# jbrea/BayesianOptimization.jl

Hardware: AMD Instinct MI355X
Metric: acquisition-candidates/sec (N=3000,d=8) (higher is better)
Workload: dtype f64

## Files before the change

### bayesianoptimization.jl_amd/csrc/bohip.hip

```cpp
#include "../../include/bohip.h"
#include "../../include/bohip_paths.h"
#include "../../include/bohip_fit.h"
#include "../../include/bohip_qei.h"
#include "../../include/bohip_acq.h"
#include "../../include/bohip_kg.h"
#include "../../include/bohip_ens.h"
#include "kernels_linalg.hip"
#include "kernels_chol.hip"
#include "kernels_exec.hip"
#include "kernels_score.hip"
#include "kernels_batch.hip"
#include "kernels_sample.hip"
#include "kernels_qei.hip"
#include "kernels_kg.hip"
#include "kernels_path.hip"
#include "kernels_ascent.hip"
#include "kernels_fit.hip"
#include "kernels_ens.hip"
#include "kernels_small.hip"
#include "direct_l.h"

#include <algorithm>
#include <atomic>
#include <chrono>
// ... 292 lines not shown
    HIPCHK(hipMalloc(&g->dr, (g->ld + 256) * 8));
    HIPCHK(hipMalloc(&g->dt, (g->ld + 256) * 8));
    HIPCHK(hipMalloc(&g->dApp, (size_t)APP_ROWS * g->ld * 8));
    {
        const size_t Tm = (size_t)(g->ld / TILE) + 1;
        HIPCHK(hipMalloc(&g->dchol_flags, chol_flag_words((int)std::min<size_t>(Tm, CHOL_DF_TCAP)) * sizeof(unsigned)));
        HIPCHK(hipMalloc(&g->dchol_idl, Tm * CH_PANELS * 256 * 8));
    }
    HIPCHK(hipMemsetAsync(g->dL, 0, mat, g->stream));
    HIPCHK(hipMemsetAsync(g->dW, 0, mat, g->stream));
    HIPCHK(hipMemsetAsync(g->dWT, 0, mat, g->stream));
    HIPCHK(hipMemsetAsync(g->dS, 0, mat, g->stream));
    if (g->n > 0) {
        HIPCHK(hipMemcpyAsync(g->dX, g->hX.data(), (size_t)g->n * g->d * 8, hipMemcpyHostToDevice, g->stream));
        HIPCHK(hipMemcpyAsync(g->dy, g->hy.data(), (size_t)g->n * 8, hipMemcpyHostToDevice, g->stream));
    }
    g->stale = true;
    return 0;
}

static int g_bulk_pieces = 4;
static int g_sample_mfma_min = 200;
static int g_path_mfma_min = 24;
static int g_split = 1;
static int g_asc_wg_nmax = 256;
static const double g_asc_first_step = 0.1;
static int g_asc_fold = 1;
static int g_asc_lockstep = 0;
static int g_small_m = 0;
static int g_small_r = -1;
static int g_inv_hi_h = 16;
static int g_chol_df = 1;
static bool g_chol_df_strict = false;
static bool g_chol_df_dump = false;
static int g_chol_df_tmax = 96;
static std::atomic<int> g_chol_df_skip{0}, g_chol_df_backoff{0};
static unsigned long long g_chol_spin_ticks = CH_SPIN_TICKS_DEFAULT;
static int g_chol_exec_patience_us = 1000;
static int g_chol_exec_fill_inv = 1;
static int g_chol_exec_inv_pairs = 0;
static std::atomic<int> g_chol_inv_grp_min{28};
static std::atomic<int> g_chol_inv_g{8};
static int g_chol_nsf = 3;
static int g_chol_exec_urgent = -1;
static int g_chol_exec_second = 1;
static int g_small_zero_copy = 1;
static int g_chol_exec_nbu = 2;
static int g_chol_exec_fast = -1;
static int g_chol_exec_pairs = -1;
static int g_chol_exec_wgs = -1;
static int g_append_alpha_inc = 1;
static int64_t g_chunk_rows_forced = 0;
static int g_prune_m = -1;
static int launch_gemm_nt(bohip_gp* g, const GemmNTParams& p, int batch = 1, hipStream_t st = nullptr, bool hi = false) {
    if (p.mt <= 0 || p.nt64 <= 0 || p.kc <= 0 || batch <= 0) return 0;
    if (hi) hipLaunchKernelGGL(k_gemm_nt_hi, dim3(p.mt * p.nt64, batch), dim3(GEMM_THREADS_8), glds3_lds_bytes<4>(), st ? st : g->stream, p);
    else hipLaunchKernelGGL(k_gemm_nt, dim3(p.mt * p.nt64, batch), dim3(GEMM_THREADS_8), glds3_lds_bytes<4>(), st ? st : g->stream, p);
    HIPCHK(hipGetLastError());
    return 0;
}

static int device_cus();
static void read_dev_knobs() {
#if BOHIP_DEV_KNOBS
    struct Knob { const char* name; int* v; int lo, hi; };
    static int chunk_rows = 0, dump = 0;
    const Knob knobs[] = {
        {"BOHIP_CHOL_DF_TMAX", &g_chol_df_tmax, 0, CHOL_DF_TCAP}, {"BOHIP_INV_HI_H", &g_inv_hi_h, 0, 1 << 20},
        {"BOHIP_CHOL_EXEC_PAIRS", &g_chol_exec_pairs, -1, 64},
        {"BOHIP_CHOL_EXEC_URGENT", &g_chol_exec_urgent, 1, 1 << 20}, {"BOHIP_CHOL_NSF", &g_chol_nsf, 1, CH_NSF_MAX},
        {"BOHIP_CHOL_EXEC_PATIENCE_US", &g_chol_exec_patience_us, 0, 1 << 30}, {"BOHIP_CHOL_EXEC_FILL_INV", &g_chol_exec_fill_inv, 0, 1},
        {"BOHIP_CHOL_EXEC_INV_PAIRS", &g_chol_exec_inv_pairs, 0, 1}, {"BOHIP_CHOL_EXEC_WGS", &g_chol_exec_wgs, 1, 1 << 20},
        {"BOHIP_CHOL_EXEC_FAST", &g_chol_exec_fast, -1, 1 << 20},
        {"BOHIP_CHOL_EXEC_SECOND", &g_chol_exec_second, 0, 1}, {"BOHIP_SMALL_ZERO_COPY", &g_small_zero_copy, 0, 1}, {"BOHIP_CHOL_EXEC_NBU", &g_chol_exec_nbu, 0, 16}, {"BOHIP_CHUNK_ROWS", &chunk_rows, 0, 1 << 30},
        {"BOHIP_PRUNE_M", &g_prune_m, -1, 1 << 16},
        {"BOHIP_APPEND_ALPHA_INC", &g_append_alpha_inc, 0, 1}, {"BOHIP_BULK_PIECES", &g_bulk_pieces, 0, 8}, {"BOHIP_SPLIT", &g_split, 0, 1},
        {"BOHIP_SMALL_R", &g_small_r, 0, SMALL_MAX}, {"BOHIP_SMALL_M", &g_small_m, 0, 1 << 20}, {"BOHIP_CHOL_DF_DUMP", &dump, 0, 1},
    };
    for (const Knob& k : knobs)
        if (const char* e = getenv(k.name)) *k.v = std::min(k.hi, std::max(k.lo, atoi(e)));
    g_chunk_rows_forced = chunk_rows;
    g_chol_df_dump = dump != 0;
#endif
}

static int one_time_kernel_setup() {
    static bool done_dev[64] = {false};
    int dev = 0;
    HIPCHK(hipGetDevice(&dev));
    bool& done = done_dev[dev & 63];
    if (done) return 0;
    HIPCHK(hipFuncSetAttribute((const void*)k_potf2_inv, hipFuncAttributeMaxDynamicSharedMemorySize, POTF2_LDS_BYTES));
    HIPCHK(hipFuncSetAttribute((const void*)k_gemm_nt, hipFuncAttributeMaxDynamicSharedMemorySize, glds3_lds_bytes<4>()));
    HIPCHK(hipFuncSetAttribute((const void*)k_trigemm_sq, hipFuncAttributeMaxDynamicSharedMemorySize, glds3_lds_bytes<4>()));
    HIPCHK(hipFuncSetAttribute((const void*)k_trigemm_rows, hipFuncAttributeMaxDynamicSharedMemorySize, RS_LDS_BYTES));
    HIPCHK(hipFuncSetAttribute((const void*)k_batch_cond<true>, hipFuncAttributeMaxDynamicSharedMemorySize, BATCH_LDS_MAX));
    HIPCHK(hipFuncSetAttribute((const void*)k_batch_cond<false>, hipFuncAttributeMaxDynamicSharedMemorySize, BATCH_LDS_MAX));
    HIPCHK(hipFuncSetAttribute((const void*)k_chol_chain, hipFuncAttributeMaxDynamicSharedMemorySize, CH_LDS_BYTES));
    HIPCHK(hipFuncSetAttribute((const void*)k_gemm_nt_hi, hipFuncAttributeMaxDynamicSharedMemorySize, glds3_lds_bytes<4>()));
    HIPCHK(hipFuncSetAttribute((const void*)k_chol_exec, hipFuncAttributeMaxDynamicSharedMemorySize, glds3_lds_bytes<4>()));
    HIPCHK(hipFuncSetAttribute((const void*)k_trimv_stream<TRIMV_D>, hipFuncAttributeMaxDynamicSharedMemorySize, trimv_lds_bytes(TRIMV_D)));
    HIPCHK(hipFuncSetAttribute((const void*)k_path_mfma<true>, hipFuncAttributeMaxDynamicSharedMemorySize, (int)path_mfma_lds_bytes(DMAX)));
    HIPCHK(hipFuncSetAttribute((const void*)k_path_mfma<false>, hipFuncAttributeMaxDynamicSharedMemorySize, (int)path_mfma_lds_bytes(DMAX)));
    HIPCHK(hipFuncSetAttribute((const void*)k_kg<true>, hipFuncAttributeMaxDynamicSharedMemorySize, (int)kg_lds_bytes(KG_RMAX)));
    HIPCHK(hipFuncSetAttribute((const void*)k_kg<false>, hipFuncAttributeMaxDynamicSharedMemorySize, (int)kg_lds_bytes(KG_RMAX)));
    if (const char* e = getenv("BOHIP_CHOL_DATAFLOW")) g_chol_df = atoi(e);
    if (const char* e = getenv("BOHIP_CHOL_SPIN_US")) g_chol_spin_ticks = 100ull * (unsigned long long)std::max(1, atoi(e));
    if (const char* e = getenv("BOHIP_CHOL_INV_G")) g_chol_inv_g = std::min(64, std::max(0, atoi(e)));
    if (const char* e = getenv("BOHIP_CHOL_INV_GRP_MIN")) g_chol_inv_grp_min = std::max(0, atoi(e));
    if (const char* e = getenv("BOHIP_ASC_WG_NMAX")) g_asc_wg_nmax = std::max(0, atoi(e));
    if (const char* e = getenv("BOHIP_ASC_LOCKSTEP")) { g_asc_lockstep = atoi(e) == 1; g_asc_fold = atoi(e) != 2; }
    if (const char* e = getenv("BOHIP_SAMPLE_MFMA_MIN")) g_sample_mfma_min = std::max(1, atoi(e));
    g_chol_df_strict = getenv("BOHIP_CHOL_DF_STRICT") != nullptr;
    read_dev_knobs();
    done = true;
    return 0;
}

static int launch_rows_trimv(bohip_gp* g, const double* W, int64_t N0, const double* rows, int P, double* out, int upper);
static int compute_alpha(bohip_gp* g) {
    const int64_t N = g->n;
    g->alpha_inc_run = 0;
    hipLaunchKernelGGL(k_sub_mean, dim3((N + 255) / 256), dim3(256), 0, g->stream, g->dy, g->beta, N, g->dr);
    HIPCHK(hipGetLastError());
    CHK(launch_rows_trimv(g, g->dW, N, g->dr, 1, g->dt, 0));
    CHK(launch_rows_trimv(g, g->dWT, N, g->dt, 1, g->dalpha, 1));
    HIPCHK(hipMemcpyAsync(g->dW + N * g->ld, g->dalpha, (size_t)N * 8, hipMemcpyDeviceToDevice, g->stream));
    return 0;
}

static int check_info(bohip_gp* g) {
    int info = 0;
    if (g->hpin) {
        int* pw = reinterpret_cast<int*>(g->hpin + 3 * SMALL_R) + 1;
        HIPCHK(hipMemcpyAsync(pw, g->dinfo, sizeof(int), hipMemcpyDeviceToHost, g->stream));
        HIPCHK(hipStreamSynchronize(g->stream));
        info = *pw;
    } else {
        HIPCHK(hipMemcpyAsync(&info, g->dinfo, sizeof(int), hipMemcpyDeviceToHost, g->stream));
        HIPCHK(hipStreamSynchronize(g->stream));
    }
    if (info != 0) {
        g->pivot = info;
        g->stale = true;
        return fail(BOHIP_E_NOTPD, "kernel matrix not positive definite at pivot " + std::to_string(info));
    }
    g->pivot = 0;
// ... 1135 lines not shown
    return 0;
}

constexpr int PRUNE_K1 = 64;
constexpr int PRUNE_ROWS_CAP = 256;
constexpr int PRUNE_R2_GROUPS = 8;
constexpr int64_t PRUNE_R_MAX = 8192;
static int prune_tiles(int T) {
    if (g_prune_m >= 0) return g_prune_m < T ? g_prune_m : 0;
    int m = 2;
    while ((double)m * (m + 1) < 0.02 * T * (T + 1)) ++m;
    return m < T ? m : 0;
}
static std::vector<int> rows_halves(const std::vector<int>& pieces) {
    std::vector<int> out;
    for (int c : pieces) {
        const int rt = c & 0xffff, mode = c >> 16;
        if (mode == PIECE_UPPER_SOLO) out.push_back(rt | 1 << 17);
        else { out.push_back(rt | 1 << 16); out.push_back(rt); }
    }
    std::stable_sort(out.begin(), out.end(), [](int a, int b) {
        return 8 * (a & 0xffff) + ((a >> 16) & 1) * 4 > 8 * (b & 0xffff) + ((b >> 16) & 1) * 4;
    });
    return out;
}
static int rows_halves_from(const std::vector<int>& hv, int t0) {
    int n = 0;
    while (n < (int)hv.size() && (hv[n] & 0xffff) >= t0) ++n;
    return n;
}
static int launch_trigemm_rows(bohip_gp* g, const double* KsT, const int* halves, int NH, const int* list, const unsigned* cnt,
                               int cnt_max, double* q, int64_t ldq, double* mu, int groups = 0, const PruneFinish* pf = nullptr,
                               unsigned* arrive = nullptr) {
    if (NH <= 0 || cnt_max <= 0) return 0;
    RowsParams rp{};
    rp.W = g->dW; rp.ldw = g->ld; rp.KsT = KsT; rp.ldk = g->ld; rp.list = list; rp.cnt = cnt; rp.cnt_max = cnt_max;
    rp.halves = halves; rp.NH = NH; rp.G = groups > 0 ? groups : (cnt_max + RS_COLS - 1) / RS_COLS;
    rp.alpha_row = g->n; rp.q = q; rp.ldq = ldq; rp.mu = mu;
    if (pf) { rp.finish = 1; rp.arrive = arrive; rp.pf = *pf; }
    hipLaunchKernelGGL(k_trigemm_rows, dim3((unsigned)(8 * ((NH + 7) / 8) * rp.G)), dim3(RS_THREADS), RS_LDS_BYTES, g->stream, rp);
    HIPCHK(hipGetLastError());
    return 0;
}
static int launch_trigemm_on(bohip_gp* g, const double* KsT, const int* pieces, int NP, int CT, double* q, int64_t ldq, double* mu_raw,
                             FuseParams fz) {
    const int n_local = (CT + 7) / 8;
    if (NP <= 0 || CT <= 0) return 0;
    if (g->timing && g->dclk) fz.clk = g->dclk;
    hipLaunchKernelGGL(k_trigemm_sq, dim3(8 * n_local * NP), dim3(GEMM_THREADS_8), glds3_lds_bytes<4>(), g->stream, g->dW, g->ld, KsT,
                       g->ld, pieces, NP, CT, g->n, q, ldq, mu_raw, (int64_t)0, nullptr, g->ld, fz);
    HIPCHK(hipGetLastError());
    return 0;
}
static int pruned_pass(bohip_gp* g, const double* dXs, int64_t R, int m, const AcqParams& ap, Best* d_best, int64_t best_off,
                       double* ub_host = nullptr, bool long_form = false) {
    CHK(one_time_kernel_setup());
    if (!g->hprune_stat) {
        HIPCHK(hipHostMalloc((void**)&g->hprune_stat, 64, hipHostMallocDefault));
        g->hprune_stat[0] = 0u;
    }
    const int64_t N = g->n, Npad = round_up(N + 1, TILE), Rpad = round_up(R, TILE) + TILE, ld = g->ld;
    const int T = (int)(Npad / TILE);
    const int64_t P = Npad / 64;
    CHK(ensure_pieces(g, T, N));
    std::vector<int> pa, pb;
    for (int c : g->hpieces) ((c & 0xffff) < m ? pa : pb).push_back(c);
    auto al = [](size_t b) { return (b + 255) / 256 * 256; };
    const size_t o_ks = 0, o_q2 = o_ks + al((size_t)Rpad * ld * 8), o_mu2 = o_q2 + al((size_t)2 * T * Rpad * 8),
                 o_ub = o_mu2 + al((size_t)Rpad * 8), o_l1 = o_ub + al((size_t)Rpad * 8), o_l2 = o_l1 + al((size_t)PRUNE_K1 * 4),
                 o_mark = o_l2 + al((size_t)Rpad * 4), o_cnt = o_mark + al((size_t)Rpad * 4), o_rec = o_cnt + 256,
                 o_parts = o_rec + 256, o_pc = o_parts + al((size_t)2 * P * Rpad * 8), total = o_pc + al((3 * g->hpieces.size() + 8) * 4);
    bool fresh = false;
    if (g->pr_bytes < total) {
        fresh = true;
        if (g->dpr) { HIPCHK(hipStreamSynchronize(g->stream)); HIPCHK(hipFree(g->dpr)); g->dpr = nullptr; g->pr_bytes = 0; }
        HIPCHK(hipMalloc(&g->dpr, total));
        g->pr_bytes = total;
    }
    char* b = g->dpr;
    double *ks2 = (double*)(b + o_ks), *q2 = (double*)(b + o_q2), *mu2 = (double*)(b + o_mu2), *ub = (double*)(b + o_ub);
    int *l1 = (int*)(b + o_l1), *l2 = (int*)(b + o_l2), *mark = (int*)(b + o_mark), *pcs = (int*)(b + o_pc);
    const KstarParts kp{g->dW + N * ld, (double*)(b + o_parts), Rpad};
    unsigned* cnt = (unsigned*)(b + o_cnt);
    Best* rec = (Best*)(b + o_rec);
    const std::vector<int> hv = rows_halves(g->hpieces);
    const int nh = rows_halves_from(hv, m);
    std::vector<int> both = pa;
    both.insert(both.end(), pb.begin(), pb.end());
    both.insert(both.end(), hv.begin(), hv.end());
    if (fresh || g->hpr_pieces != both || g->pr_pieces_at != pcs) {
        g->pr_pieces_at = pcs;
        g->hpr_pieces = both;
        HIPCHK(hipMemcpyAsync(pcs, g->hpr_pieces.data(), both.size() * sizeof(int), hipMemcpyHostToDevice, g->stream));
    }
    if (g->timing && !g->dclk) {
        HIPCHK(hipMalloc(&g->dclk, 2 * sizeof(unsigned long long)));
        HIPCHK(hipMemsetAsync(g->dclk, 0, 2 * sizeof(unsigned long long), g->stream));
    }
    g->q_tiles = T;
    g->score_launches = 1;
    const KernelHyper hp = make_hyper(g);
    const double sigma2 = std::exp(2.0 * g->logsig);
    const int k1 = (int)std::min<int64_t>(PRUNE_K1, R);
    t_begin(g, "kstar");
    CHK(launch_kstar_any(g, dXs, 0, R, Npad, hp, &kp));
    t_end(g);
    t_begin(g, "trigemm_sq");
    FuseParams fz{};
    fz.T = T;
    CHK(launch_trigemm_on(g, g->dKsT, pcs, (int)pa.size(), (int)((R + CTILE - 1) / CTILE), g->dq, Rpad, g->dmu_raw, fz));
    PruneBound bd{};
    bd.parts = kp.parts; bd.P = P; bd.ldp = Rpad; bd.Npad = Npad; bd.q = g->dq; bd.ldq = Rpad; bd.R = R; bd.m = m;
    bd.sigma2 = sigma2; bd.beta = g->beta; bd.ap = ap; bd.ub = ub;
    hipLaunchKernelGGL(k_prune_bound, dim3((unsigned)((R + 63) / 64)), dim3(64), 0, g->stream, bd);
    if (ub_host) {
        t_end(g);
        HIPCHK(hipGetLastError());
        HIPCHK(hipMemcpyAsync(ub_host, ub, (size_t)R * 8, hipMemcpyDeviceToHost, g->stream));
        HIPCHK(hipStreamSynchronize(g->stream));
        return 0;
    }
    static_assert(PRUNE_R_MAX <= (int64_t)SELECT_THREADS * SELECT_PER, "k_prune_select holds the whole batch in one workgroup");
    hipLaunchKernelGGL(k_prune_select, dim3(1), dim3(SELECT_THREADS), 0, g->stream, (const double*)ub, R, k1, l1, mark, cnt, rec);
    HIPCHK(hipGetLastError());
    PruneFinish pf{};
    pf.q = g->dq; pf.ldq = Rpad; pf.q2 = q2; pf.ldq2 = Rpad; pf.mu2 = mu2; pf.m = m; pf.T = T; pf.sigma2 = sigma2; pf.beta = g->beta;
    pf.ap = ap; pf.rec = rec;
    const int* hvd = pcs + pa.size() + pb.size();
    pf.ub = ub; pf.mark = mark; pf.R = R; pf.cnt2 = cnt + 1; pf.best_off = (long long)best_off;
    pf.list = l1; pf.cnt = cnt; pf.list2 = l2; pf.best_out = d_best; pf.stat = g->hprune_stat;
    CHK(launch_trigemm_rows(g, g->dKsT, hvd, nh, l1, cnt, k1, q2, Rpad, mu2, 0, &pf, cnt + PRUNE_ARRIVE));
    const int64_t cap = R - k1;
    pf.list = l2; pf.cnt = cnt + 1; pf.list2 = nullptr;
    if (cap > 0 && !long_form) {
        CHK(launch_trigemm_rows(g, g->dKsT, hvd, nh, l2, cnt + 1, INT_MAX, q2, Rpad, mu2, PRUNE_R2_GROUPS, &pf, cnt + PRUNE_ARRIVE + 1));
    } else if (cap > 0) {
        if (cap > PRUNE_ROWS_CAP) {
            hipLaunchKernelGGL(k_prune_gather, dim3((unsigned)cap), dim3(256), 0, g->stream, (const int*)l2, (const unsigned*)(cnt + 1),
                               (const double*)g->dKsT, ld, Npad, ks2, PRUNE_ROWS_CAP, cnt + 2);
            fz.live = cnt + 2;
            CHK(launch_trigemm_on(g, ks2, pcs + pa.size(), (int)pb.size(), (int)((cap + CTILE - 1) / CTILE), q2, Rpad, mu2, fz));
        }
        CHK(launch_trigemm_rows(g, g->dKsT, hvd, nh, l2, cnt + 1, (int)std::min<int64_t>(cap, PRUNE_ROWS_CAP), q2, Rpad, mu2));
        hipLaunchKernelGGL(k_prune_finish, dim3(1), dim3(256), 0, g->stream, pf);
        HIPCHK(hipGetLastError());
    }
    t_end(g);
    return 0;
}

constexpr int PRUNE_BACKOFF = 31;
static bool prune_wanted(bohip_gp* g, int64_t R) {
    if (g->prune_skip > 0) { --g->prune_skip; return false; }
    g->prune_seen = 0u;
    if (g->hprune_stat) {
        const unsigned n2 = __atomic_load_n(g->hprune_stat, __ATOMIC_RELAXED);
        g->prune_seen = n2;
        if ((int64_t)n2 > R / 8) {
            __atomic_store_n(g->hprune_stat, 0u, __ATOMIC_RELAXED);
            g->prune_skip = PRUNE_BACKOFF - 1;
            g->prune_retry = true;
            return false;
        }
// ... 2065 lines not shown
extern "C" {
int bohip_debug_read_w(bohip_gp* g, int which, double* out) {
    if (!g || !out) return BOHIP_E_ARG;
    hipSetDevice(g->device);
    hipStreamSynchronize(g->stream);
    const double* src = which ? g->dWT : g->dW;
    return hipMemcpy2D(out, (size_t)g->n * 8, src, (size_t)g->ld * 8, (size_t)g->n * 8, (size_t)g->n, hipMemcpyDeviceToHost) == hipSuccess ? 0 : BOHIP_E_HIP;
}
int64_t bohip_debug_exec_tasks(int T, int64_t ld, uint64_t base_L, uint64_t base_S, uint64_t base_W, uint64_t base_WT, int inv_g, uint64_t* out,
                               int64_t cap, int* qbeg, int64_t* layout) {
    std::vector<bohip::ExTask> all;
    int qb[bohip::EX_NQ + 1];
    unsigned* fb = reinterpret_cast<unsigned*>(uintptr_t(1) << 40);
    const int nsf = g_chol_nsf;
    int grp_min = g_chol_inv_grp_min;
    if (const char* e = getenv("BOHIP_CHOL_INV_GRP_MIN")) grp_min = std::max(0, atoi(e));
    exec_task_list(reinterpret_cast<double*>(base_L), reinterpret_cast<double*>(base_S), reinterpret_cast<double*>(base_W),
                   reinterpret_cast<double*>(base_WT), fb, ld, T, nsf, inv_g, all, qb, grp_min);
    for (int i = 0; i <= bohip::EX_NQ; ++i) qbeg[i] = qb[i];
    const bohip::CholFlags fl = chol_flags_layout_at(fb, nullptr, T);
    const unsigned* ptrs[10] = {fl.panel, fl.solved, fl.crit, fl.rest, fl.col, fl.farall, fl.fol, fl.colall, fl.colr, fl.xp};
    for (int i = 0; i < 10; ++i) layout[i] = ptrs[i] - fb;
    layout[10] = nsf;
    layout[11] = (int64_t)chol_inv_word(T);
    layout[12] = (int64_t)chol_xp3_word(T);
    layout[13] = exec_bulk_stride_ok(all, qb, 4) ? 2 : 1;
    if ((int64_t)all.size() <= cap && out) std::memcpy(out, all.data(), all.size() * sizeof(bohip::ExTask));
    return (int64_t)all.size();
}
int bohip_debug_trigemm_pieces(int T, int64_t alpha_row, int* out, int cap) {
    one_time_kernel_setup();
    std::vector<int> ps;
    trigemm_pieces(T, alpha_row, ps);
    for (int i = 0; i < (int)ps.size() && i < cap; ++i) out[i] = ps[i];
    return (int)ps.size();
}
int bohip_debug_prune_bounds(bohip_gp* g, int acq_id, const double* acq_params, const double* Xs, int64_t R, double* ub) {
    if (!g || R <= 0 || !Xs || !ub || !acq_id_scores(acq_id)) return fail(BOHIP_E_ARG, "bad arguments");
    HIPCHK(hipSetDevice(g->device));
    if (g->n == 0) return fail(BOHIP_E_STATE, "model has no observations");
    CHK(ensure_fresh(g));
    CHK(ensure_xs(g, R));
    CHK(ensure_score_scratch(g, R));
    static const double no_params[2] = {0.0, 0.0};
    AcqParams ap;
    CHK(make_acq(acq_id, acq_params ? acq_params : no_params, &ap));
    const int m = prune_tiles((int)(round_up(g->n + 1, TILE) / TILE));
    if (m == 0 || R > PRUNE_R_MAX || R > g->chunk_now || (path_R(g, R) <= small_limit(g) && R <= SMALL_MAX) || split_plan(g, R).nsl > 0)
        return fail(BOHIP_E_UNSUPPORTED, "no pruning at this size");
    HIPCHK(hipMemcpyAsync(g->dXs, Xs, (size_t)R * g->d * 8, hipMemcpyHostToDevice, g->stream));
    return pruned_pass(g, g->dXs, R, m, ap, nullptr, 0, ub);
}
int bohip_debug_trigemm_partials(bohip_gp* g, const double* Xs, int64_t R, int path, double* q_out, double* mu_out) {
    if (!g || R <= 0 || !Xs || !q_out || !mu_out || path < 0 || path > 2) return fail(BOHIP_E_ARG, "bad arguments");
    HIPCHK(hipSetDevice(g->device));
    if (g->n == 0) return fail(BOHIP_E_STATE, "model has no observations");
    CHK(ensure_fresh(g));
    CHK(ensure_xs(g, R));
    CHK(ensure_score_scratch(g, R));
    if (R > g->chunk_now) return fail(BOHIP_E_UNSUPPORTED, "more than one K*' chunk");
    CHK(one_time_kernel_setup());
    const int64_t N = g->n, Npad = round_up(N + 1, TILE), Rpad = round_up(R, TILE);
    const int T = (int)(Npad / TILE);
    CHK(ensure_pieces(g, T, N));
    const std::vector<int> hv = rows_halves(g->hpieces);
    HIPCHK(hipMemcpyAsync(g->dXs, Xs, (size_t)R * g->d * 8, hipMemcpyHostToDevice, g->stream));
    CHK(launch_kstar_any(g, g->dXs, 0, R, Npad, make_hyper(g)));
    std::vector<double> q((size_t)2 * T * Rpad), mu((size_t)Rpad);
    if (path == 0) {
        CHK(launch_trigemm_on(g, g->dKsT, g->dpieces, g->n_pieces, (int)((R + CTILE - 1) / CTILE), g->dq, Rpad, g->dmu_raw, FuseParams{}));
        HIPCHK(hipMemcpyAsync(q.data(), g->dq, q.size() * 8, hipMemcpyDeviceToHost, g->stream));
        HIPCHK(hipMemcpyAsync(mu.data(), g->dmu_raw, mu.size() * 8, hipMemcpyDeviceToHost, g->stream));
        HIPCHK(hipStreamSynchronize(g->stream));
        for (int t = 0; t < 2 * T; ++t) std::memcpy(q_out + (size_t)t * R, q.data() + (size_t)t * Rpad, (size_t)R * 8);
        std::memcpy(mu_out, mu.data(), (size_t)R * 8);
        return 0;
    }
    std::vector<int> list((size_t)R);
    for (int64_t i = 0; i < R; ++i) list[i] = (int)(R - 1 - i);
    const unsigned n = (unsigned)R;
    char* d = nullptr;
    const size_t o_q = 0, o_mu = o_q + q.size() * 8, o_l = o_mu + mu.size() * 8, o_h = o_l + list.size() * 4, o_c = o_h + hv.size() * 4;
    HIPCHK(hipMalloc(&d, o_c + 16));
    int rc = 0;
    hipMemcpyAsync(d + o_l, list.data(), list.size() * 4, hipMemcpyHostToDevice, g->stream);
    hipMemcpyAsync(d + o_h, hv.data(), hv.size() * 4, hipMemcpyHostToDevice, g->stream);
    hipMemcpyAsync(d + o_c, &n, 4, hipMemcpyHostToDevice, g->stream);
    rc = launch_trigemm_rows(g, g->dKsT, (const int*)(d + o_h), (int)hv.size(), (const int*)(d + o_l), (const unsigned*)(d + o_c), (int)R,
                             (double*)(d + o_q), Rpad, (double*)(d + o_mu), path == 2 ? 1 : 0);
    hipMemcpyAsync(q.data(), d + o_q, q.size() * 8, hipMemcpyDeviceToHost, g->stream);
    hipMemcpyAsync(mu.data(), d + o_mu, mu.size() * 8, hipMemcpyDeviceToHost, g->stream);
    const hipError_t e = hipStreamSynchronize(g->stream);
    hipFree(d);
    if (rc != 0) return rc;
    if (e != hipSuccess) return fail(BOHIP_E_HIP, hipGetErrorString(e));
    for (int t = 0; t < 2 * T; ++t)
        for (int64_t i = 0; i < R; ++i) q_out[(size_t)t * R + list[i]] = q[(size_t)t * Rpad + i];
    for (int64_t i = 0; i < R; ++i) mu_out[list[i]] = mu[i];
    return 0;
}
int64_t bohip_debug_prune_stat(bohip_gp* g) {
    if (!g || !g->hprune_stat) return -1;
    return (int64_t)__atomic_load_n(g->hprune_stat, __ATOMIC_RELAXED);
}
int bohip_debug_prune_round2_form(bohip_gp* g, int form) {
    if (!g || form < -1 || form > 1) return fail(BOHIP_E_ARG, "bad arguments");
    g->prune_r2_form = form;
    return 0;
}
int bohip_debug_set_chol_inv_g(int g_new) {
    return g_chol_inv_g.exchange(std::min(64, std::max(0, g_new)));
}
int bohip_debug_exec_throughput(bohip_gp* g, unsigned qmask, int hot, int wgs, double* ms_out, double* gflop_out) {
    if (!g || !ms_out || g->n == 0) return BOHIP_E_ARG;
    hipSetDevice(g->device);
    CHK(one_time_kernel_setup());
    const int T = (int)(round_up(g->n + 1, TILE) / TILE);
    if (T <= 3) return BOHIP_E_UNSUPPORTED;
    std::vector<ExTask> all, run;
    int qb[EX_NQ + 1], qb2[EX_NQ + 1];
    exec_task_list(g->dL, g->dS, g->dW, g->dWT, g->dchol_flags, g->ld, T, g_chol_nsf, g_chol_inv_g, all, qb);
    double fl = 0.0;
    qb2[0] = 0;
    for (int qi = 0; qi < EX_NQ; ++qi) {
        if ((qmask >> qi) & 1u)
            for (int i = qb[qi]; i < qb[qi + 1]; ++i) {
                ExTask t = all[i];
                for (int d = 0; d < EX_NDEP; ++d) { t.dep_idx[d] = EX_NONE; t.dep_want[d] = 0; }
// ... 63 lines not shown
```

### bayesianoptimization.jl_amd/csrc/gemm_core.h

```cpp
#pragma once
#ifndef BOHIP_TRACE
#define BOHIP_TRACE 0
#endif
#ifndef BOHIP_ABL
#define BOHIP_ABL 0
#endif
#include <type_traits>
#include "common.h"

namespace bohip {

typedef double d2 __attribute__((ext_vector_type(2)));

__device__ __forceinline__ double mfma444(double a, double b, double c) {
    return __builtin_amdgcn_mfma_f64_4x4x4f64(a, b, c, 0, 0, 0);
}

typedef __attribute__((address_space(3))) void* lds_void_ptr;
typedef const __attribute__((address_space(1))) void* gbl_void_ptr;
constexpr int GL_ROW = KC;

template <int NJ>
__device__ __forceinline__ void load_frags_swz(const double* ap, const double* bp, const int (&oa)[2], const int (&ob)[2],
                                               int S, d2 (&av)[8], d2 (&bv)[NJ]) {
// ... 36 lines not shown
template <int NJ>
__device__ __forceinline__ void mma_chunk_swz(const double* ap, const double* bp, const int (&oa)[2], const int (&ob)[2],
                                              double (&acc)[8][NJ]) {
    d2 a0[8], b0[NJ], a1[8], b1[NJ];
    load_frags_swz<NJ>(ap, bp, oa, ob, 0, a0, b0);
    __builtin_amdgcn_sched_barrier(0);
    load_frags_swz<NJ>(ap, bp, oa, ob, 1, a1, b1);
    __builtin_amdgcn_sched_barrier(0);
    mma_pair<NJ>(a0, b0, acc);
    __builtin_amdgcn_sched_barrier(0);
    mma_pair<NJ>(a1, b1, acc);
}

template <int NJ>
constexpr int glds3_lds_bytes() { return 3 * (TILE + 16 * NJ) * GL_ROW * 8; }

template <int NJ, int ABL, int XY>
__device__ __forceinline__ void chunk_mma(const double* ap, const double* bp, int skip, double (&acc)[8][NJ]) {
    d2 av[8], bv[NJ];
    const uint32_t pa = (uint32_t)(uintptr_t)(__attribute__((address_space(3))) const double*)ap;
    const uint32_t pb = (uint32_t)(uintptr_t)(__attribute__((address_space(3))) const double*)bp;
    if constexpr ((ABL & 2) != 0) {
#pragma unroll
        for (int j = 0; j < NJ; ++j) asm volatile("" : "=v"(bv[j]) : "v"(pb));
#pragma unroll
        for (int i = 0; i < 8; ++i) asm volatile("" : "=v"(av[i]) : "v"(pa));
    } else {
        bv[0] = ds_read128<0>(pb); bv[1] = ds_read128<1024>(pb); bv[2] = ds_read128<2048>(pb); bv[3] = ds_read128<3072>(pb);
        av[0] = ds_read128<0>(pa); av[1] = ds_read128<1024>(pa); av[2] = ds_read128<2048>(pa); av[3] = ds_read128<3072>(pa);
        av[4] = ds_read128<4096>(pa); av[5] = ds_read128<5120>(pa); av[6] = ds_read128<6144>(pa); av[7] = ds_read128<7168>(pa);
    }
    asm volatile("s_waitcnt lgkmcnt(7)" : "+v"(bv[0]), "+v"(bv[1]), "+v"(bv[2]), "+v"(bv[3]), "+v"(av[0]));
    if (skip <= 0) mma_row<NJ, XY>(av[0], bv, acc[0]);
    asm volatile("s_waitcnt lgkmcnt(6)" : "+v"(av[1]));
    if (skip <= 1) mma_row<NJ, XY>(av[1], bv, acc[1]);
    asm volatile("s_waitcnt lgkmcnt(5)" : "+v"(av[2]));
    if (skip <= 2) mma_row<NJ, XY>(av[2], bv, acc[2]);
    asm volatile("s_waitcnt lgkmcnt(4)" : "+v"(av[3]));
    if (skip <= 3) mma_row<NJ, XY>(av[3], bv, acc[3]);
    asm volatile("s_waitcnt lgkmcnt(3)" : "+v"(av[4]));
    if (skip <= 4) mma_row<NJ, XY>(av[4], bv, acc[4]);
    asm volatile("s_waitcnt lgkmcnt(2)" : "+v"(av[5]));
    if (skip <= 5) mma_row<NJ, XY>(av[5], bv, acc[5]);
    asm volatile("s_waitcnt lgkmcnt(1)" : "+v"(av[6]));
    if (skip <= 6) mma_row<NJ, XY>(av[6], bv, acc[6]);
    asm volatile("s_waitcnt lgkmcnt(0)" : "+v"(av[7]));
    if (skip <= 7) mma_row<NJ, XY>(av[7], bv, acc[7]);
}

constexpr int GEMM_THREADS_8 = 512;
#if BOHIP_TRACE
__device__ unsigned long long g_phase[8192 * 8 * 4];
#endif
template <int NJ, int ABL = 0, bool SWAVE = false, bool FOLD = true>
__device__ __forceinline__ void gemm_tile_loop_glds3_ks(const double* __restrict__ A, int64_t lda,
                                                        const double* __restrict__ B, int64_t ldb, int kc_begin,
                                                        int kc_end, double* smem, double (&acc)[8][NJ],
                                                        int active_rows = TILE, int tri_kc = 1 << 30, int tid_in = -1) {
    static_assert(NJ == 4, "piece distribution below assumes 16 + 8 DMA pieces per chunk");
    constexpr int AT = TILE * GL_ROW, BT = 16 * NJ * GL_ROW;
    const int tid = tid_in >= 0 ? tid_in : (int)threadIdx.x, lane = tid & 63, wave = SWAVE ? __builtin_amdgcn_readfirstlane(tid >> 6) : (tid >> 6);
    const int khalf = wave >> 2, w4 = wave & 3, wr = w4 >> 1, wc = w4 & 1;
    double* As = smem;
    double* Bs = smem + 3 * AT;
    if (kc_begin >= kc_end) return;
    const int prow = lane >> 3, sseg = (lane & 7) ^ (lane >> 3);
    const double* a_src0 = A + (int64_t)(wave * 8 + prow) * lda + sseg * 2;
    const double* a_src1 = A + (int64_t)((wave + 8) * 8 + prow) * lda + sseg * 2;
    const double* b_src = B + (int64_t)(wave * 8 + prow) * ldb + sseg * 2;
    double* a_dst0 = As + wave * 8 * GL_ROW;
    double* a_dst1 = As + (wave + 8) * 8 * GL_ROW;
    double* b_dst = Bs + wave * 8 * GL_ROW;
    auto issue = [&](int kc, int buf) {
        __builtin_amdgcn_global_load_lds((gbl_void_ptr)(a_src0 + (int64_t)kc * KC), (lds_void_ptr)(a_dst0 + buf * AT), 16, 0, 0);
        __builtin_amdgcn_global_load_lds((gbl_void_ptr)(a_src1 + (int64_t)kc * KC), (lds_void_ptr)(a_dst1 + buf * AT), 16, 0, 0);
        __builtin_amdgcn_global_load_lds((gbl_void_ptr)(b_src + (int64_t)kc * KC), (lds_void_ptr)(b_dst + buf * BT), 16, 0, 0);
    };
    auto issue_h = [&](int kc, int buf) {
        __builtin_amdgcn_global_load_lds((gbl_void_ptr)(a_src0 + (int64_t)kc * KC), (lds_void_ptr)(a_dst0 + buf * AT), 16, 0, 0);
        __builtin_amdgcn_global_load_lds((gbl_void_ptr)(b_src + (int64_t)kc * KC), (lds_void_ptr)(b_dst + buf * BT), 16, 0, 0);
    };
    const int k = lane >> 4, b = (lane >> 2) & 3, t = lane & 3;
    const int r7a = 4 * (b >> 1) + t, r7b = 4 * (b & 1) + t;
    const int oa = ((4 * khalf + k) ^ r7a) << 1, ob = ((4 * khalf + k) ^ r7b) << 1;
    const bool half = active_rows <= TILE / 2;
    const int wre = half ? 0 : wr;
    const int xy = __builtin_amdgcn_readfirstlane(half ? 1 + wr : 0);
    const int a_frag = (wre * 64 + r7a) * GL_ROW + oa, b_frag = (wc * 8 * NJ + r7b) * GL_ROW + ob;
    const bool wave_active = half || wr * 64 < active_rows;
    const int skip0 = __builtin_amdgcn_readfirstlane(khalf - 8 * wre);
    if (half) {
        issue_h(kc_begin, 0);
        if (kc_begin + 1 < kc_end) {
            issue_h(kc_begin + 1, 1);
            asm volatile("s_waitcnt vmcnt(2)" ::: "memory");
        } else {
            asm volatile("s_waitcnt vmcnt(0)" ::: "memory");
        }
    } else {
        issue(kc_begin, 0);
        if (kc_begin + 1 < kc_end) {
            issue(kc_begin + 1, 1);
            asm volatile("s_waitcnt vmcnt(3)" ::: "memory");
        } else {
            asm volatile("s_waitcnt vmcnt(0)" ::: "memory");
        }
    }
    __builtin_amdgcn_s_barrier();
    auto run = [&](auto xy_tag) {
        int cur = 0;
#if BOHIP_TRACE
        unsigned long long ph0 = 0, ph1 = 0, ph2 = 0, phn = 0;
#endif
        for (int kc = kc_begin; kc < kc_end; ++kc) {
#if BOHIP_TRACE
            const unsigned long long tA = __builtin_amdgcn_s_memtime();
#endif
            const int nxt2 = cur == 0 ? 2 : cur - 1;
            const bool more2 = kc + 2 < kc_end;
            constexpr bool HALF = decltype(xy_tag)::value != 0;
            if (more2 && !(ABL & 1)) {
                if constexpr (HALF) issue_h(kc + 2, nxt2);
                else issue(kc + 2, nxt2);
            }
            if (wave_active) {
                const double* ap = As + cur * AT + a_frag;
                const double* bp = Bs + cur * BT + b_frag;
                const int skip = kc >= tri_kc ? 2 * (kc - tri_kc) + skip0 : 0;
                chunk_mma<NJ, ABL, decltype(xy_tag)::value>(ap, bp, skip, acc);
            }
            __builtin_amdgcn_sched_barrier(0);
#if BOHIP_TRACE
            const unsigned long long tB = __builtin_amdgcn_s_memtime();
            __builtin_amdgcn_sched_barrier(0);
#endif
            if (more2) {
                if constexpr (HALF) asm volatile("s_waitcnt vmcnt(2)" ::: "memory");
                else asm volatile("s_waitcnt vmcnt(3)" ::: "memory");
            } else {
                asm volatile("s_waitcnt vmcnt(0)" ::: "memory");
            }
            asm volatile("s_waitcnt lgkmcnt(0)" ::: "memory");
#if BOHIP_TRACE
            const unsigned long long tC = __builtin_amdgcn_s_memtime();
            __builtin_amdgcn_sched_barrier(0);
#endif
            if constexpr ((ABL & 4) == 0) __builtin_amdgcn_s_barrier();
            __builtin_amdgcn_sched_barrier(0);
#if BOHIP_TRACE
            const unsigned long long tD = __builtin_amdgcn_s_memtime();
            ph0 += tB - tA; ph1 += tC - tB; ph2 += tD - tC; phn += 1;
#endif
            cur = cur == 2 ? 0 : cur + 1;
        }
#if BOHIP_TRACE
        if (lane == 0 && blockIdx.x < 8192) {
            unsigned long long* o = g_phase + ((size_t)blockIdx.x * 8 + wave) * 4;
            o[0] = ph0; o[1] = ph1; o[2] = ph2; o[3] = phn;
        }
#endif
    };
    if (xy == 0) run(std::integral_constant<int, 0>{});
    else if (xy == 1) run(std::integral_constant<int, 1>{});
    else run(std::integral_constant<int, 2>{});
    if constexpr (!FOLD) return;
    double* xch = smem;
    if (khalf == 1) {
#pragma unroll
        for (int i = 0; i < 8; ++i)
#pragma unroll
            for (int j = 0; j < NJ; ++j) xch[(i * NJ + j) * 256 + (tid & 255)] = acc[i][j];
    }
    __syncthreads();
    if (khalf == 0) {
#pragma unroll
        for (int i = 0; i < 8; ++i)
#pragma unroll
            for (int j = 0; j < NJ; ++j) acc[i][j] += xch[(i * NJ + j) * 256 + tid];
    }
    __syncthreads();
    if (half) {
        if (khalf == 0 && wr == 1) {
#pragma unroll
            for (int i = 0; i < 8; ++i)
#pragma unroll
                for (int j = 0; j < NJ; ++j) {
                    xch[(i * NJ + j) * 256 + (tid - 128)] = acc[i][j];
                    acc[i][j] = 0.0;
                }
        }
        __syncthreads();
        if (khalf == 0 && wr == 0) {
#pragma unroll
            for (int i = 0; i < 8; ++i)
#pragma unroll
                for (int j = 0; j < NJ; ++j) acc[i][j] += xch[(i * NJ + j) * 256 + tid];
        }
        __syncthreads();
    }
}

__device__ __forceinline__ int acc_row(int lane, int wr, int mi) {
    return wr * 64 + 8 * mi + 4 * (((lane >> 2) & 3) >> 1) + (lane >> 4);
}
template <int NJ>
__device__ __forceinline__ int acc_col(int lane, int wc, int nj) {
    return wc * 8 * NJ + 8 * nj + 4 * (((lane >> 2) & 3) & 1) + (lane & 3);
}

}
```

### bayesianoptimization.jl_amd/csrc/kernels_score.hip

```cpp
#include "gemm_core.h"
#include "acq_log.h"

namespace bohip {

template <bool LOW>
__device__ __forceinline__ double cov_from_r_fast(int fam, double sigma2, double r) {
    if constexpr (LOW) {
        return matern_lo_k(fam, sigma2, r);
    } else {
        if (fam == FAM_M52) {
            const double R = sqrt(r), s = sqrt(5.0) * R;
            return sigma2 * (1.0 + s + 5.0 / 3.0 * r) * exp(-s);
        }
        return sigma2 * exp(-0.5 * r);
    }
}

struct KstarParts {
    const double* alpha;
    double* parts;
    int64_t ldp;
};
__device__ __forceinline__ void swap32(double a, double b, double& x, double& y) {
    const unsigned long long ua = (unsigned long long)__double_as_longlong(a), ub = (unsigned long long)__double_as_longlong(b);
// ... 199 lines not shown
    __syncthreads();
    if (tid < 2 * CW) {
        const int hh = tid >> 6, c = tid & (CW - 1);
        double* dst = q_part + (int64_t)(2 * rt + (mode == PIECE_WHOLE ? hh : 0)) * ldq + r_off + (int64_t)ct * CW + c;
        if (mode == PIECE_WHOLE || hh == 0) __hip_atomic_store(dst, red[hh * CW + c], __ATOMIC_RELAXED, __HIP_MEMORY_SCOPE_AGENT);
        else __hip_atomic_store(dst + ldq, 0.0, __ATOMIC_RELAXED, __HIP_MEMORY_SCOPE_AGENT);
    }
    if (fz.tile_cnt != nullptr) {
        __shared__ int s_last;
        const int tile_g = (int)(r_off / CW) + ct;
        asm volatile("s_waitcnt vmcnt(0)" ::: "memory");
        __syncthreads();
        if (tid == 0) s_last = atomicAdd(fz.tile_cnt + tile_g, 1u) == (unsigned)(NP - 1);
        __syncthreads();
        if (s_last && tid < 64) trigemm_fused_finish(fz, tile_g, fz.T, q_part, ldq, mu_raw);
    }
}

__global__ __launch_bounds__(GEMM_THREADS_8, 4) void k_trigemm_sq(const double* __restrict__ W, int64_t ldw,
                                                                  const double* __restrict__ KsT, int64_t ldk,
                                                                  const int* __restrict__ pieces, int NP, int CT, int64_t alpha_row,
                                                                  double* __restrict__ q_part, int64_t ldq,
                                                                  double* __restrict__ mu_raw, int64_t r_off,
                                                                  double* __restrict__ VT, int64_t ldv, FuseParams fz) {
    extern __shared__ __attribute__((aligned(16))) double smem[];
#if BOHIP_TRACE
    const unsigned long long t_start = wall_clock64(), c_start = clock64();
    struct TraceEnd {
        unsigned long long t0, c0;
        __device__ ~TraceEnd() {
            if (threadIdx.x == 0) {
                unsigned hw, xcc;
                asm volatile("s_getreg_b32 %0, hwreg(HW_REG_HW_ID)" : "=s"(hw));
                asm volatile("s_getreg_b32 %0, hwreg(HW_REG_XCC_ID)" : "=s"(xcc));
                unsigned long long* t = g_trace + 6 * (size_t)blockIdx.x;
                t[0] = t0; t[1] = wall_clock64(); t[2] = hw; t[3] = xcc; t[4] = c0; t[5] = clock64();
            }
        }
    } trace_end{t_start, c_start};
#endif
    const int xcd = blockIdx.x & 7, slot = blockIdx.x >> 3;
    const int n_local = (CT + 7) >> 3;
    const int ct = xcd + 8 * (slot % n_local);
    if (ct >= CT) return;
    if (fz.live != nullptr && ct * CTILE >= (int)*fz.live) return;
    const int piece = __builtin_amdgcn_readfirstlane(pieces[slot / n_local]);
    __shared__ unsigned long long s_clk[2];
    if (fz.clk != nullptr && blockIdx.x % 33 == 0 && threadIdx.x == 0) { s_clk[0] = clock64(); s_clk[1] = wall_clock64(); }
    trigemm_job(piece & 0xffff, piece >> 16, ct, W, ldw, KsT, ldk, NP, alpha_row, q_part, ldq, mu_raw, r_off, VT, ldv, fz, smem,
                    (int)threadIdx.x);
    if (fz.clk != nullptr && blockIdx.x % 33 == 0 && threadIdx.x == 0) {
        atomicAdd(fz.clk, (unsigned long long)clock64() - s_clk[0]);
        atomicAdd(fz.clk + 1, (unsigned long long)wall_clock64() - s_clk[1]);
    }
}

__global__ __launch_bounds__(256) void k_split_combine_v(const double* __restrict__ PT, int64_t plane, int64_t ldp, int kz,
                                                         int64_t N, double* __restrict__ q, double* __restrict__ mu_raw,
                                                         double* __restrict__ VT, int64_t ldv) {
    __shared__ double red[256];
    const int r = blockIdx.x;
    const double* base = PT + (int64_t)r * ldp;
    double s = 0.0;
    for (int64_t i = threadIdx.x; i <= N; i += 256) {
        const int nsl = (int)(((i >> 7) + 1) * (TILE / KC) + kz - 1) / kz;
        double v = 0.0;
        for (int sl = 0; sl < nsl; ++sl) v += base[(int64_t)sl * plane + i];
        if (i < N) {
            s += v * v;
            if (VT) VT[(int64_t)r * ldv + i] = v;
        } else {
            mu_raw[r] = v;
        }
    }
    red[threadIdx.x] = s;
    __syncthreads();
    for (int o = 128; o > 0; o >>= 1) {
        if (threadIdx.x < o) red[threadIdx.x] += red[threadIdx.x + o];
        __syncthreads();
    }
    if (threadIdx.x == 0) q[r] = red[0];
}
__global__ __launch_bounds__(256) void k_split_combine_u(const double* __restrict__ PU, int64_t plane, int64_t ldp, int kz,
                                                         int nslices, int64_t N, double* __restrict__ UT, int64_t ldu) {
    const int r = blockIdx.x;
    const double* base = PU + (int64_t)r * ldp;
    for (int64_t j = threadIdx.x; j < N; j += 256) {
        const int s0 = (int)((j >> 7) * (TILE / KC)) / kz;
        double v = 0.0;
        for (int sl = s0; sl < nslices; ++sl) v += base[(int64_t)sl * plane + j];
        UT[(int64_t)r * ldu + j] = v;
    }
}

template <bool LOGEI = true>
__device__ __forceinline__ double acq_eval(const AcqParams& a, double mu, double s2) {
#pragma clang fp contract(off)
    switch (a.acq) {
        case ACQ_EI: {
            const double tau = a.p0;
            if (s2 == 0.0) return mu > tau ? mu - tau : 0.0;
            const double D = mu - tau;
            const double cdf = 1.0 / 2.0 * (1.0 + erf(D / sqrt(2.0 * s2)));
            const double pdf = 1.0 / sqrt(2.0 * M_PI * s2) * exp(-(D * D) / (2.0 * s2));
            return D * cdf + sqrt(s2) * pdf;
        }
// ... 857 lines not shown
```

Baseline: 26.44 million.

## Split pruned-pass phase-A triangular GEMM into 64-row half jobs with reordered schedule

Phase A of the pruned pass now launches a dedicated kernel in which each whole row tile of the prefix is split into two 64-row jobs. Each job covers only its triangular k-range, so the top half stops early. The GEMM core gains a ROWS64 mode that splits k across wave pairs instead of rows. Jobs are sorted by cost and partly rotated to balance load across workgroups. This aims to cut wasted triangular work and tail imbalance, at the price of doubling the block count and adding extra fold/reduction synchronisation.

Result: faster. 28.52 million, median of 6 (+7.9%).

```diff
diff --git a/bayesianoptimization.jl_amd/csrc/bohip.hip b/bayesianoptimization.jl_amd/csrc/bohip.hip
--- a/bayesianoptimization.jl_amd/csrc/bohip.hip
+++ b/bayesianoptimization.jl_amd/csrc/bohip.hip
@@ -368,6 +368,7 @@
 static int g_append_alpha_inc = 1;
 static int64_t g_chunk_rows_forced = 0;
 static int g_prune_m = -1;
+static int g_pa_order = 1;
 static int launch_gemm_nt(bohip_gp* g, const GemmNTParams& p, int batch = 1, hipStream_t st = nullptr, bool hi = false) {
     if (p.mt <= 0 || p.nt64 <= 0 || p.kc <= 0 || batch <= 0) return 0;
     if (hi) hipLaunchKernelGGL(k_gemm_nt_hi, dim3(p.mt * p.nt64, batch), dim3(GEMM_THREADS_8), glds3_lds_bytes<4>(), st ? st : g->stream, p);
@@ -389,7 +390,7 @@
         {"BOHIP_CHOL_EXEC_INV_PAIRS", &g_chol_exec_inv_pairs, 0, 1}, {"BOHIP_CHOL_EXEC_WGS", &g_chol_exec_wgs, 1, 1 << 20},
         {"BOHIP_CHOL_EXEC_FAST", &g_chol_exec_fast, -1, 1 << 20},
         {"BOHIP_CHOL_EXEC_SECOND", &g_chol_exec_second, 0, 1}, {"BOHIP_SMALL_ZERO_COPY", &g_small_zero_copy, 0, 1}, {"BOHIP_CHOL_EXEC_NBU", &g_chol_exec_nbu, 0, 16}, {"BOHIP_CHUNK_ROWS", &chunk_rows, 0, 1 << 30},
-        {"BOHIP_PRUNE_M", &g_prune_m, -1, 1 << 16},
+        {"BOHIP_PRUNE_M", &g_prune_m, -1, 1 << 16}, {"BOHIP_PA_ORDER", &g_pa_order, 0, 1},
         {"BOHIP_APPEND_ALPHA_INC", &g_append_alpha_inc, 0, 1}, {"BOHIP_BULK_PIECES", &g_bulk_pieces, 0, 8}, {"BOHIP_SPLIT", &g_split, 0, 1},
         {"BOHIP_SMALL_R", &g_small_r, 0, SMALL_MAX}, {"BOHIP_SMALL_M", &g_small_m, 0, 1 << 20}, {"BOHIP_CHOL_DF_DUMP", &dump, 0, 1},
     };
@@ -409,6 +410,7 @@
     HIPCHK(hipFuncSetAttribute((const void*)k_potf2_inv, hipFuncAttributeMaxDynamicSharedMemorySize, POTF2_LDS_BYTES));
     HIPCHK(hipFuncSetAttribute((const void*)k_gemm_nt, hipFuncAttributeMaxDynamicSharedMemorySize, glds3_lds_bytes<4>()));
     HIPCHK(hipFuncSetAttribute((const void*)k_trigemm_sq, hipFuncAttributeMaxDynamicSharedMemorySize, glds3_lds_bytes<4>()));
+    HIPCHK(hipFuncSetAttribute((const void*)k_trigemm_sq_pa, hipFuncAttributeMaxDynamicSharedMemorySize, glds3_lds_bytes<4>()));
     HIPCHK(hipFuncSetAttribute((const void*)k_trigemm_rows, hipFuncAttributeMaxDynamicSharedMemorySize, RS_LDS_BYTES));
     HIPCHK(hipFuncSetAttribute((const void*)k_batch_cond<true>, hipFuncAttributeMaxDynamicSharedMemorySize, BATCH_LDS_MAX));
     HIPCHK(hipFuncSetAttribute((const void*)k_batch_cond<false>, hipFuncAttributeMaxDynamicSharedMemorySize, BATCH_LDS_MAX));
@@ -1650,6 +1652,24 @@
     HIPCHK(hipGetLastError());
     return 0;
 }
+static std::vector<int> phase_a_jobs(const std::vector<int>& pieces, int m) {
+    std::vector<int> out;
+    for (int c : pieces)
+        if ((c & 0xffff) < m) { out.push_back((c & 0xffff) | 1 << 16); out.push_back(c & 0xffff); }
+    std::stable_sort(out.begin(), out.end(), [](int a, int b) {
+        return 8 * (a & 0xffff) + (a >> 16) * 4 > 8 * (b & 0xffff) + (b >> 16) * 4;
+    });
+    if (g_pa_order == 1) std::rotate(out.begin(), out.begin() + out.size() / 3, out.begin() + 2 * (out.size() / 3));
+    return out;
+}
+static int launch_phase_a(bohip_gp* g, const double* KsT, const int* jobs, int NJOBS, int CT, double* q, int64_t ldq) {
+    const int n_local = (CT + 7) / 8;
+    if (NJOBS <= 0 || CT <= 0) return 0;
+    hipLaunchKernelGGL(k_trigemm_sq_pa, dim3(8 * n_local * NJOBS), dim3(GEMM_THREADS_8), glds3_lds_bytes<4>(), g->stream, g->dW, g->ld,
+                       KsT, g->ld, jobs, CT, q, ldq, g->timing && g->dclk ? g->dclk : nullptr);
+    HIPCHK(hipGetLastError());
+    return 0;
+}
 static int pruned_pass(bohip_gp* g, const double* dXs, int64_t R, int m, const AcqParams& ap, Best* d_best, int64_t best_off,
                        double* ub_host = nullptr, bool long_form = false) {
     CHK(one_time_kernel_setup());
@@ -1663,11 +1683,15 @@
     CHK(ensure_pieces(g, T, N));
     std::vector<int> pa, pb;
     for (int c : g->hpieces) ((c & 0xffff) < m ? pa : pb).push_back(c);
+    if (m >= T) return fail(BOHIP_E_STATE, "pruned pass: the prefix holds the alpha row");
+    for (int c : pa)
+        if (c >> 16 != PIECE_WHOLE) return fail(BOHIP_E_STATE, "pruned pass: a half piece in the prefix");
+    const std::vector<int> ph = phase_a_jobs(g->hpieces, m);
     auto al = [](size_t b) { return (b + 255) / 256 * 256; };
     const size_t o_ks = 0, o_q2 = o_ks + al((size_t)Rpad * ld * 8), o_mu2 = o_q2 + al((size_t)2 * T * Rpad * 8),
                  o_ub = o_mu2 + al((size_t)Rpad * 8), o_l1 = o_ub + al((size_t)Rpad * 8), o_l2 = o_l1 + al((size_t)PRUNE_K1 * 4),
                  o_mark = o_l2 + al((size_t)Rpad * 4), o_cnt = o_mark + al((size_t)Rpad * 4), o_rec = o_cnt + 256,
-                 o_parts = o_rec + 256, o_pc = o_parts + al((size_t)2 * P * Rpad * 8), total = o_pc + al((3 * g->hpieces.size() + 8) * 4);
+                 o_parts = o_rec + 256, o_pc = o_parts + al((size_t)2 * P * Rpad * 8), total = o_pc + al((5 * g->hpieces.size() + 8) * 4);
     bool fresh = false;
     if (g->pr_bytes < total) {
         fresh = true;
@@ -1686,6 +1710,7 @@
     std::vector<int> both = pa;
     both.insert(both.end(), pb.begin(), pb.end());
     both.insert(both.end(), hv.begin(), hv.end());
+    both.insert(both.end(), ph.begin(), ph.end());
     if (fresh || g->hpr_pieces != both || g->pr_pieces_at != pcs) {
         g->pr_pieces_at = pcs;
         g->hpr_pieces = both;
@@ -1706,7 +1731,7 @@
     t_begin(g, "trigemm_sq");
     FuseParams fz{};
     fz.T = T;
-    CHK(launch_trigemm_on(g, g->dKsT, pcs, (int)pa.size(), (int)((R + CTILE - 1) / CTILE), g->dq, Rpad, g->dmu_raw, fz));
+    CHK(launch_phase_a(g, g->dKsT, pcs + pa.size() + pb.size() + hv.size(), (int)ph.size(), (int)((R + CTILE - 1) / CTILE), g->dq, Rpad));
     PruneBound bd{};
     bd.parts = kp.parts; bd.P = P; bd.ldp = Rpad; bd.Npad = Npad; bd.q = g->dq; bd.ldq = Rpad; bd.R = R; bd.m = m;
     bd.sigma2 = sigma2; bd.beta = g->beta; bd.ap = ap; bd.ub = ub;
@@ -3878,7 +3903,7 @@
     return pruned_pass(g, g->dXs, R, m, ap, nullptr, 0, ub);
 }
 int bohip_debug_trigemm_partials(bohip_gp* g, const double* Xs, int64_t R, int path, double* q_out, double* mu_out) {
-    if (!g || R <= 0 || !Xs || !q_out || !mu_out || path < 0 || path > 2) return fail(BOHIP_E_ARG, "bad arguments");
+    if (!g || R <= 0 || !Xs || !q_out || !mu_out || path < 0 || path > 3) return fail(BOHIP_E_ARG, "bad arguments");
     HIPCHK(hipSetDevice(g->device));
     if (g->n == 0) return fail(BOHIP_E_STATE, "model has no observations");
     CHK(ensure_fresh(g));
@@ -3900,6 +3925,24 @@
         HIPCHK(hipStreamSynchronize(g->stream));
         for (int t = 0; t < 2 * T; ++t) std::memcpy(q_out + (size_t)t * R, q.data() + (size_t)t * Rpad, (size_t)R * 8);
         std::memcpy(mu_out, mu.data(), (size_t)R * 8);
+        return 0;
+    }
+    if (path == 3) {
+        const int m = prune_tiles(T);
+        if (m <= 0 || m >= T) return fail(BOHIP_E_UNSUPPORTED, "no pruning at this size");
+        const std::vector<int> ph = phase_a_jobs(g->hpieces, m);
+        int* dj = nullptr;
+        HIPCHK(hipMalloc(&dj, ph.size() * sizeof(int)));
+        hipMemcpyAsync(dj, ph.data(), ph.size() * sizeof(int), hipMemcpyHostToDevice, g->stream);
+        hipMemsetAsync(g->dq, 0, q.size() * 8, g->stream);
+        const int rc = launch_phase_a(g, g->dKsT, dj, (int)ph.size(), (int)((R + CTILE - 1) / CTILE), g->dq, Rpad);
+        hipMemcpyAsync(q.data(), g->dq, q.size() * 8, hipMemcpyDeviceToHost, g->stream);
+        const hipError_t e = hipStreamSynchronize(g->stream);
+        hipFree(dj);
+        if (rc != 0) return rc;
+        if (e != hipSuccess) return fail(BOHIP_E_HIP, hipGetErrorString(e));
+        for (int t = 0; t < 2 * T; ++t) std::memcpy(q_out + (size_t)t * R, q.data() + (size_t)t * Rpad, (size_t)R * 8);
+        std::memset(mu_out, 0, (size_t)R * 8);
         return 0;
     }
     std::vector<int> list((size_t)R);
diff --git a/bayesianoptimization.jl_amd/csrc/gemm_core.h b/bayesianoptimization.jl_amd/csrc/gemm_core.h
--- a/bayesianoptimization.jl_amd/csrc/gemm_core.h
+++ b/bayesianoptimization.jl_amd/csrc/gemm_core.h
@@ -112,15 +112,17 @@
 #if BOHIP_TRACE
 __device__ unsigned long long g_phase[8192 * 8 * 4];
 #endif
-template <int NJ, int ABL = 0, bool SWAVE = false, bool FOLD = true>
+template <int NJ, int ABL = 0, bool SWAVE = false, bool FOLD = true, bool ROWS64 = false>
 __device__ __forceinline__ void gemm_tile_loop_glds3_ks(const double* __restrict__ A, int64_t lda,
                                                         const double* __restrict__ B, int64_t ldb, int kc_begin,
                                                         int kc_end, double* smem, double (&acc)[8][NJ],
-                                                        int active_rows = TILE, int tri_kc = 1 << 30, int tid_in = -1) {
+                                                        int active_rows = TILE, int tri_kc = 1 << 30, int tid_in = -1,
+                                                        int row_h = 0) {
     static_assert(NJ == 4, "piece distribution below assumes 16 + 8 DMA pieces per chunk");
     constexpr int AT = TILE * GL_ROW, BT = 16 * NJ * GL_ROW;
     const int tid = tid_in >= 0 ? tid_in : (int)threadIdx.x, lane = tid & 63, wave = SWAVE ? __builtin_amdgcn_readfirstlane(tid >> 6) : (tid >> 6);
-    const int khalf = wave >> 2, w4 = wave & 3, wr = w4 >> 1, wc = w4 & 1;
+    const int w4 = wave & 3;
+    const int khalf = ROWS64 ? w4 >> 1 : wave >> 2, wr = ROWS64 ? wave >> 2 : w4 >> 1, wc = w4 & 1;
     double* As = smem;
     double* Bs = smem + 3 * AT;
     if (kc_begin >= kc_end) return;
@@ -143,13 +145,13 @@
     const int k = lane >> 4, b = (lane >> 2) & 3, t = lane & 3;
     const int r7a = 4 * (b >> 1) + t, r7b = 4 * (b & 1) + t;
     const int oa = ((4 * khalf + k) ^ r7a) << 1, ob = ((4 * khalf + k) ^ r7b) << 1;
-    const bool half = active_rows <= TILE / 2;
-    const int wre = half ? 0 : wr;
+    const bool half = !ROWS64 && active_rows <= TILE / 2;
+    const int wre = half || ROWS64 ? 0 : wr;
     const int xy = __builtin_amdgcn_readfirstlane(half ? 1 + wr : 0);
     const int a_frag = (wre * 64 + r7a) * GL_ROW + oa, b_frag = (wc * 8 * NJ + r7b) * GL_ROW + ob;
-    const bool wave_active = half || wr * 64 < active_rows;
-    const int skip0 = __builtin_amdgcn_readfirstlane(khalf - 8 * wre);
-    if (half) {
+    const bool wave_active = ROWS64 ? wr == 0 : half || wr * 64 < active_rows;
+    const int skip0 = __builtin_amdgcn_readfirstlane(khalf - 8 * (ROWS64 ? row_h : wre));
+    if (half || ROWS64) {
         issue_h(kc_begin, 0);
         if (kc_begin + 1 < kc_end) {
             issue_h(kc_begin + 1, 1);
@@ -178,7 +180,7 @@
 #endif
             const int nxt2 = cur == 0 ? 2 : cur - 1;
             const bool more2 = kc + 2 < kc_end;
-            constexpr bool HALF = decltype(xy_tag)::value != 0;
+            constexpr bool HALF = decltype(xy_tag)::value != 0 || ROWS64;
             if (more2 && !(ABL & 1)) {
                 if constexpr (HALF) issue_h(kc + 2, nxt2);
                 else issue(kc + 2, nxt2);
@@ -220,23 +222,28 @@
         }
 #endif
     };
-    if (xy == 0) run(std::integral_constant<int, 0>{});
-    else if (xy == 1) run(std::integral_constant<int, 1>{});
-    else run(std::integral_constant<int, 2>{});
+    if constexpr (ROWS64) {
+        run(std::integral_constant<int, 0>{});
+    } else {
+        if (xy == 0) run(std::integral_constant<int, 0>{});
+        else if (xy == 1) run(std::integral_constant<int, 1>{});
+        else run(std::integral_constant<int, 2>{});
+    }
     if constexpr (!FOLD) return;
     double* xch = smem;
-    if (khalf == 1) {
+    const bool folds = !ROWS64 || wr == 0;
+    if (khalf == 1 && folds) {
 #pragma unroll
         for (int i = 0; i < 8; ++i)
 #pragma unroll
-            for (int j = 0; j < NJ; ++j) xch[(i * NJ + j) * 256 + (tid & 255)] = acc[i][j];
+            for (int j = 0; j < NJ; ++j) xch[(i * NJ + j) * 256 + (ROWS64 ? wc * 64 + lane : (tid & 255))] = acc[i][j];
     }
     __syncthreads();
-    if (khalf == 0) {
+    if (khalf == 0 && folds) {
 #pragma unroll
         for (int i = 0; i < 8; ++i)
 #pragma unroll
-            for (int j = 0; j < NJ; ++j) acc[i][j] += xch[(i * NJ + j) * 256 + tid];
+            for (int j = 0; j < NJ; ++j) acc[i][j] += xch[(i * NJ + j) * 256 + (ROWS64 ? wc * 64 + lane : tid)];
     }
     __syncthreads();
     if (half) {
diff --git a/bayesianoptimization.jl_amd/csrc/kernels_score.hip b/bayesianoptimization.jl_amd/csrc/kernels_score.hip
--- a/bayesianoptimization.jl_amd/csrc/kernels_score.hip
+++ b/bayesianoptimization.jl_amd/csrc/kernels_score.hip
@@ -275,6 +275,72 @@
     if (fz.clk != nullptr && blockIdx.x % 33 == 0 && threadIdx.x == 0) {
         atomicAdd(fz.clk, (unsigned long long)clock64() - s_clk[0]);
         atomicAdd(fz.clk + 1, (unsigned long long)wall_clock64() - s_clk[1]);
+    }
+}
+
+__device__ __forceinline__ void trigemm_job_rows64(int rt, int hh, int ct, const double* __restrict__ W, int64_t ldw,
+                                                   const double* __restrict__ KsT, int64_t ldk, double* __restrict__ q_part,
+                                                   int64_t ldq, double* smem, int tid) {
+    constexpr int NJ = 4, CW = CTILE;
+    double acc[8][NJ];
+#pragma unroll
+    for (int i = 0; i < 8; ++i)
+#pragma unroll
+        for (int j = 0; j < NJ; ++j) acc[i][j] = 0.0;
+    const int64_t row_base = (int64_t)rt * TILE + 64 * hh;
+    const int tri_kc = rt * (TILE / KC);
+    const int kc_end = tri_kc + (hh == 0 ? 4 : 8);
+    gemm_tile_loop_glds3_ks<NJ, BOHIP_ABL, true, true, true>(W + row_base * ldw, ldw, KsT + (int64_t)ct * CW * ldk, ldk, 0, kc_end, smem,
+                                                             acc, TILE / 2, tri_kc, tid, hh);
+    const int lane = tid & 63, wave = tid >> 6, wc = wave & 1;
+    __syncthreads();
+    double* red = smem;
+    if (wave < 2) {
+#pragma unroll
+        for (int nj = 0; nj < NJ; ++nj) {
+            double s = 0.0;
+#pragma unroll
+            for (int mi = 0; mi < 8; ++mi) s = sq_step(s, acc[mi][nj]);
+            s = sq_tree(s);
+            if (lane < 8) red[wc * 8 * NJ + 8 * nj + lane] = s;
+        }
+    }
+    __syncthreads();
+    if (tid < CW)
+        __hip_atomic_store(q_part + (int64_t)(2 * rt + hh) * ldq + (int64_t)ct * CW + tid, red[tid], __ATOMIC_RELAXED, __HIP_MEMORY_SCOPE_AGENT);
+}
+
+__global__ __launch_bounds__(GEMM_THREADS_8, 4) void k_trigemm_sq_pa(const double* __restrict__ W, int64_t ldw,
+                                                                     const double* __restrict__ KsT, int64_t ldk,
+                                                                     const int* __restrict__ jobs, int CT, double* __restrict__ q_part,
+                                                                     int64_t ldq, unsigned long long* clk) {
+    extern __shared__ __attribute__((aligned(16))) double smem[];
+#if BOHIP_TRACE
+    const unsigned long long t_start = wall_clock64(), c_start = clock64();
+    struct TraceEnd {
+        unsigned long long t0, c0;
+        __device__ ~TraceEnd() {
+            if (threadIdx.x == 0) {
+                unsigned hw, xcc;
+                asm volatile("s_getreg_b32 %0, hwreg(HW_REG_HW_ID)" : "=s"(hw));
+                asm volatile("s_getreg_b32 %0, hwreg(HW_REG_XCC_ID)" : "=s"(xcc));
+                unsigned long long* t = g_trace + 6 * (size_t)blockIdx.x;
+                t[0] = t0; t[1] = wall_clock64(); t[2] = hw; t[3] = xcc; t[4] = c0; t[5] = clock64();
+            }
+        }
+    } trace_end{t_start, c_start};
+#endif
+    const int xcd = blockIdx.x & 7, slot = blockIdx.x >> 3;
+    const int n_local = (CT + 7) >> 3;
+    const int ct = xcd + 8 * (slot % n_local);
+    if (ct >= CT) return;
+    const int job = __builtin_amdgcn_readfirstlane(jobs[slot / n_local]);
+    __shared__ unsigned long long s_clk[2];
+    if (clk != nullptr && blockIdx.x % 33 == 0 && threadIdx.x == 0) { s_clk[0] = clock64(); s_clk[1] = wall_clock64(); }
+    trigemm_job_rows64(job & 0xffff, job >> 16, ct, W, ldw, KsT, ldk, q_part, ldq, smem, (int)threadIdx.x);
+    if (clk != nullptr && blockIdx.x % 33 == 0 && threadIdx.x == 0) {
+        atomicAdd(clk, (unsigned long long)clock64() - s_clk[0]);
+        atomicAdd(clk + 1, (unsigned long long)wall_clock64() - s_clk[1]);
     }
 }
 
```
